# tobwei/APTAI

Measured on AMD Instinct MI355X. Metric: utterances/sec (10 s @ 16 kHz) train-step, higher is better.
Workload: dtype bf16

## Files before the change

### aptai_amd/csrc/attention.hip

```cpp
#include "common.h"

namespace {

#ifdef APTAI_STAMPS
__device__ unsigned long long g_attn_stamps[3 * 1024 * 8];
#define ATTN_STAMP(k, slot)                                                                                       \
    do {                                                                                                          \
        if (threadIdx.x == 0) {                                                                                   \
            const int bl = blockIdx.x + gridDim.x * (blockIdx.y + gridDim.y * blockIdx.z);                        \
            if (bl < 1024) g_attn_stamps[((k) * 1024 + bl) * 8 + (slot)] = wall_clock64();                         \
        }                                                                                                         \
    } while (0)
#else
#define ATTN_STAMP(k, slot) do {} while (0)
#endif

constexpr int HD = 64;
constexpr float LOG2E = 1.4426950408889634f;

struct AttnArgs {
    const bf16_t* qkv; long ld;
    const int* lens;
    bf16_t* ctx; long ldo;
    float* lse2;
// ... 12 lines not shown
    int q_prescaled;
};

__device__ __forceinline__ int tile_swz(int row) { return ((row >> 2) & 3) | (((row >> 1) & 1) << 2); }
__device__ __forceinline__ int tile_off(int row, int chunk) { return row * 128 + ((chunk ^ tile_swz(row)) << 4); }

struct LaneOffs {
    int rowk[4];
    int tr[2][2];
};
__device__ __forceinline__ LaneOffs lane_offs(int lane) {
    LaneOffs o;
    const int r31 = lane & 31, h = lane >> 5;
#pragma unroll
    for (int ds = 0; ds < 4; ++ds) o.rowk[ds] = tile_off(r31, 2 * ds + h);
    const int dgrp = (lane >> 4) & 1, i = lane & 15, qq = i >> 2, p = i & 3;
    const int trow = 4 * h + qq;
#pragma unroll
    for (int dt = 0; dt < 2; ++dt)
#pragma unroll
        for (int hi = 0; hi < 2; ++hi) o.tr[dt][hi] = tile_off(trow + 8 * hi, dt * 4 + 2 * dgrp + (p >> 1)) + ((p & 1) << 3);
    return o;
}
__device__ __forceinline__ bf16x8 rd_row(const char* tile, const LaneOffs& o, int row_block, int ds) {
    return *(const bf16x8*)(tile + o.rowk[ds] + row_block * 4096);
}
__device__ __forceinline__ bf16x8 rd_tr(const char* tile, const LaneOffs& o, int s, int dt) {
    short4v lo = __builtin_amdgcn_ds_read_tr16_b64_v4i16((__attribute__((address_space(3))) short4v*)(tile + o.tr[dt][0] + s * 2048));
    short4v hi = __builtin_amdgcn_ds_read_tr16_b64_v4i16((__attribute__((address_space(3))) short4v*)(tile + o.tr[dt][1] + s * 2048));
    short8v r = {lo[0], lo[1], lo[2], lo[3], hi[0], hi[1], hi[2], hi[3]};
    return __builtin_bit_cast(bf16x8, r);
}

__device__ __forceinline__ bf16x8 pack8(const float* v) {
    u32x4 u = {pack2bf(v[0], v[1]), pack2bf(v[2], v[3]), pack2bf(v[4], v[5]), pack2bf(v[6], v[7])};
    return __builtin_bit_cast(bf16x8, u);
}

__device__ __forceinline__ int acc_row(int r, int h) { return (r & 3) + 8 * (r >> 2) + 4 * h; }

constexpr int OUT_PITCH = 144;
constexpr int STAGE_BYTES = 4 * 32 * OUT_PITCH;
constexpr int DQ_STAGE = 2 * 128 * 128;
constexpr int DKDV_BLOCKS = 3;
constexpr int DKDV_KV_BYTES = 2 * 128 * 128;

__device__ __forceinline__ void stage_rows128(char* dst, const bf16_t* src, long ld, int tid) {
#pragma unroll
    for (int it = 0; it < 4; ++it) {
        const int cid = it * 256 + tid, row = cid >> 3, ch = cid & 7;
        *(u32x4*)(dst + tile_off(row, ch)) = *(const u32x4*)(src + (long)row * ld + ch * 8);
    }
}
__device__ __forceinline__ void store_rows_bf16(char* sw, const f32x16 (&acc)[2], float scale, bf16_t* g_row0, long ld, int lane) {
    const int r31 = lane & 31, h = lane >> 5;
#pragma unroll
    for (int dt = 0; dt < 2; ++dt)
#pragma unroll
        for (int g4 = 0; g4 < 4; ++g4) {
            const int d = dt * 32 + 8 * g4 + 4 * h;
            *(u32x2*)(sw + r31 * OUT_PITCH + d * 2) = (u32x2){pack2bf(acc[dt][4 * g4] * scale, acc[dt][4 * g4 + 1] * scale),
                                                              pack2bf(acc[dt][4 * g4 + 2] * scale, acc[dt][4 * g4 + 3] * scale)};
        }
    __builtin_amdgcn_fence(__ATOMIC_RELEASE, "wavefront");
#pragma unroll
    for (int i = 0; i < 4; ++i) {
        const int idx = i * 64 + lane, r = idx >> 3, ch = idx & 7;
        *(u32x4*)(g_row0 + (long)r * ld + ch * 8) = *(const u32x4*)(sw + r * OUT_PITCH + ch * 16);
    }
    __builtin_amdgcn_fence(__ATOMIC_ACQUIRE, "wavefront");
}

__device__ __forceinline__ bool attn_keep(uint32_t pair, int key, uint32_t s0, uint32_t s1, uint32_t thr16) {
    const uint32_t hsh = rng_hash(pair, s0, s1);
    return ((key & 1) ? (hsh >> 16) : (hsh & 0xffffu)) >= thr16;
}

__device__ __forceinline__ void attn_block(const AttnArgs& a, int& tile, int& hd, int& b) {
    const int nt = gridDim.x, total = nt * gridDim.y * gridDim.z;
    int L = blockIdx.x + nt * (blockIdx.y + gridDim.y * blockIdx.z);
    if (a.xcd_remap && (total & 7) == 0) L = (L & 7) * (total >> 3) + (L >> 3);
    tile = L % nt;
    const int grp = L / nt;
    hd = grp % (int)gridDim.y;
    b = grp / (int)gridDim.y;
}

constexpr int FWD_BUF = 2 * 64 * 128;
constexpr int FWD_SMEM = 2 * FWD_BUF;
constexpr float REF_HEADROOM = 40.0f;
constexpr float REF_SUM_LIMIT = 1.4901161193847656e-08f;

template <bool V> struct Flag { static constexpr bool value = V; };

template <bool DROP>
__global__ __launch_bounds__(256, 3) void attn_fwd_kernel(AttnArgs a) {
    __shared__ __attribute__((aligned(16))) char smem[FWD_SMEM];
    ATTN_STAMP(0, 0);
    if (DROP) apply_salt(a.salt, a.seed0, a.seed1);
    const int tid = threadIdx.x, lane = tid & 63, wave = tid >> 6, h = lane >> 5;
    int tile_x, hd, b;
    attn_block(a, tile_x, hd, b);
    const int q0 = tile_x * 128 + wave * 32;
    int len = a.lens[b];
    len = len < 1 ? 1 : (len > a.Tp ? a.Tp : len);
    const int ntiles = (len + 63) >> 6;
    const long rowbase = (long)b * a.Tp;
    const int q = q0 + (lane & 31);
    const bf16_t* Qg = a.qkv + (rowbase + q) * a.ld + hd * HD;
    const bf16_t* Kg = a.qkv + rowbase * a.ld + a.H + hd * HD;
    const bf16_t* Vg = Kg + a.H;
    const LaneOffs lo = lane_offs(lane);

    bf16x8 qf[4];
#pragma unroll
    for (int ds = 0; ds < 4; ++ds) qf[ds] = *(const bf16x8*)(Qg + ds * 16 + h * 8);
    __builtin_amdgcn_sched_barrier(0);

    f32x16 oT[2];
    oT[0] = (f32x16)(0.f);
    oT[1] = (f32x16)(0.f);
    float ref = 0.f, l_run = 0.f;

    int soff[2];
    long goff[2];
#pragma unroll
    for (int it = 0; it < 2; ++it) {
        const int cid = it * 256 + tid, row = cid >> 3, ch = cid & 7;
        soff[it] = tile_off(row, ch);
        goff[it] = (long)row * a.ld + ch * 8;
    }
    u32x4 kreg[2], vreg[2];
    const long tile_stride = 64 * a.ld;
#pragma unroll
    for (int it = 0; it < 2; ++it) { kreg[it] = *(const u32x4*)(Kg + goff[it]); vreg[it] = *(const u32x4*)(Vg + goff[it]); }
    uint32_t hbase = 0;
    if (DROP) hbase = rng_hash((uint32_t)((b * a.heads + hd) * a.Tp + q), a.seed0, a.seed1) + (uint32_t)(2 * h) * ATTN_K1;
    const float c = a.c;
#pragma unroll
    for (int it = 0; it < 2; ++it) { *(u32x4*)(smem + soff[it]) = kreg[it]; *(u32x4*)(smem + 64 * 128 + soff[it]) = vreg[it]; }
    if (ntiles > 1) {
#pragma unroll
        for (int it = 0; it < 2; ++it) {
            kreg[it] = *(const u32x4*)(Kg + tile_stride + goff[it]);
            vreg[it] = *(const u32x4*)(Vg + tile_stride + goff[it]);
        }
    }
    __syncthreads();
    ATTN_STAMP(0, 1);

    auto tile = [&](auto first_flag, auto mask_flag, const int t) {
        constexpr bool FIRST = decltype(first_flag)::value, MASK = decltype(mask_flag)::value;
        const char* sK = smem + (t & 1) * FWD_BUF;
        const char* sV = sK + 64 * 128;
        const int kbase = t * 64;
        bf16x8 kfr[2][4];
#pragma unroll
        for (int ds = 0; ds < 4; ++ds) kfr[0][ds] = rd_row(sK, lo, 0, ds);
        if (t + 1 < ntiles) {
            char* nb = smem + ((t + 1) & 1) * FWD_BUF;
#pragma unroll
            for (int it = 0; it < 2; ++it) { *(u32x4*)(nb + soff[it]) = kreg[it]; *(u32x4*)(nb + 64 * 128 + soff[it]) = vreg[it]; }
            if (t + 2 < ntiles) {
                const bf16_t* kn = Kg + (long)(t + 2) * tile_stride;
                const bf16_t* vn = Vg + (long)(t + 2) * tile_stride;
#pragma unroll
                for (int it = 0; it < 2; ++it) { kreg[it] = *(const u32x4*)(kn + goff[it]); vreg[it] = *(const u32x4*)(vn + goff[it]); }
            }
        }
        f32x16 sT[2];
        sT[0] = __builtin_amdgcn_mfma_f32_32x32x16_bf16(kfr[0][0], qf[0], (f32x16)(0.f), 0, 0, 0);
#pragma unroll
        for (int ds = 1; ds < 4; ++ds) sT[0] = __builtin_amdgcn_mfma_f32_32x32x16_bf16(kfr[0][ds], qf[ds], sT[0], 0, 0, 0);
#pragma unroll
        for (int ds = 0; ds < 4; ++ds) kfr[1][ds] = rd_row(sK, lo, 1, ds);
        sT[1] = __builtin_amdgcn_mfma_f32_32x32x16_bf16(kfr[1][0], qf[0], (f32x16)(0.f), 0, 0, 0);
#pragma unroll
        for (int ds = 1; ds < 4; ++ds) sT[1] = __builtin_amdgcn_mfma_f32_32x32x16_bf16(kfr[1][ds], qf[ds], sT[1], 0, 0, 0);
        if (MASK) {
#pragma unroll
            for (int kt2 = 0; kt2 < 2; ++kt2)
#pragma unroll
                for (int r = 0; r < 16; ++r)
                    if (kbase + kt2 * 32 + acc_row(r, h) >= len) sT[kt2][r] = -INFINITY;
        }
        if (FIRST) {
            float mt = sT[0][0];
#pragma unroll
            for (int r = 1; r < 16; ++r) mt = fmaxf(mt, sT[0][r]);
#pragma unroll
            for (int r = 0; r < 16; ++r) mt = fmaxf(mt, sT[1][r]);
            mt = fmaxf(mt, __shfl_xor(mt, 32, 64));
            ref = fmaf(mt, c, REF_HEADROOM);
        }
        float psum = 0.f;
#pragma unroll
        for (int kt2 = 0; kt2 < 2; ++kt2) {
            bf16x8 vfr[2][2];
#pragma unroll
            for (int s = 0; s < 2; ++s)
#pragma unroll
                for (int dt = 0; dt < 2; ++dt) vfr[s][dt] = rd_tr(sV, lo, 2 * kt2 + s, dt);
            float x[16];
#pragma unroll
            for (int r = 0; r < 16; ++r) { x[r] = fast_exp2(fmaf(sT[kt2][r], c, -ref)); psum += x[r]; }
            if (DROP) {
#pragma unroll
                for (int r = 0; r < 16; r += 2) {
                    const uint32_t hsh = attn_mix(hbase + (uint32_t)(kbase / 2 + 16 * kt2 + acc_row(r, 0) / 2) * ATTN_K1);
                    x[r] = (hsh & 0xffffu) >= a.thr16 ? x[r] : 0.f;
                    x[r + 1] = (hsh >> 16) >= a.thr16 ? x[r + 1] : 0.f;
                }
            }
            const bf16x8 pf0 = pack8(&x[0]), pf1 = pack8(&x[8]);
#pragma unroll
            for (int dt = 0; dt < 2; ++dt) oT[dt] = __builtin_amdgcn_mfma_f32_32x32x16_bf16(vfr[0][dt], pf0, oT[dt], 0, 0, 0);
#pragma unroll
            for (int dt = 0; dt < 2; ++dt) oT[dt] = __builtin_amdgcn_mfma_f32_32x32x16_bf16(vfr[1][dt], pf1, oT[dt], 0, 0, 0);
        }
        psum += __shfl_xor(psum, 32, 64);
        l_run += psum;
        if (!FIRST && __builtin_amdgcn_ballot_w64(!(psum <= REF_SUM_LIMIT))) {
            if (!(psum <= REF_SUM_LIMIT)) {
                const float e = floorf(fast_log2(psum)) + REF_HEADROOM;
                const float sc = fast_exp2(-e);
                ref += e;
                l_run *= sc;
#pragma unroll
                for (int r = 0; r < 16; ++r) { oT[0][r] *= sc; oT[1][r] *= sc; }
            }
        }
        __syncthreads();
    };
    if (ntiles == 1) {
        tile(Flag<true>{}, Flag<true>{}, 0);
    } else {
        tile(Flag<true>{}, Flag<false>{}, 0);
        for (int t = 1; t + 1 < ntiles; ++t) tile(Flag<false>{}, Flag<false>{}, t);
        tile(Flag<false>{}, Flag<true>{}, ntiles - 1);
    }
    ATTN_STAMP(0, 2);
    const float l_tot = l_run;
    const float inv = __frcp_rn(l_tot) * a.dscale;
    if (a.lse2 && h == 0) a.lse2[((long)b * a.heads + hd) * a.Tp + q] = ref + fast_log2(l_tot);
    char* sw = smem + wave * (32 * OUT_PITCH);
    const int r31 = lane & 31;
#pragma unroll
    for (int dt = 0; dt < 2; ++dt)
#pragma unroll
        for (int g4 = 0; g4 < 4; ++g4) {
            oT[dt][4 * g4 + 0] *= inv; oT[dt][4 * g4 + 1] *= inv; oT[dt][4 * g4 + 2] *= inv; oT[dt][4 * g4 + 3] *= inv;
            const int d = dt * 32 + 8 * g4 + 4 * h;
            *(u32x2*)(sw + r31 * OUT_PITCH + d * 2) = (u32x2){pack2bf(oT[dt][4 * g4], oT[dt][4 * g4 + 1]),
                                                              pack2bf(oT[dt][4 * g4 + 2], oT[dt][4 * g4 + 3])};
        }
    __syncthreads();
    const long orow = (rowbase + q0) * a.ldo + hd * HD;
#pragma unroll
    for (int i = 0; i < 4; ++i) {
        const int idx = i * 64 + lane, r = idx >> 3, ch = idx & 7;
        *(u32x4*)(a.ctx + orow + (long)r * a.ldo + ch * 8) = *(const u32x4*)(sw + r * OUT_PITCH + ch * 16);
    }
    if (a.o32) {
#pragma unroll
        for (int dt = 0; dt < 2; ++dt) {
            __syncthreads();
#pragma unroll
            for (int g4 = 0; g4 < 4; ++g4)
                *(f32x4*)(sw + r31 * OUT_PITCH + (8 * g4 + 4 * h) * 4) =
                    (f32x4){oT[dt][4 * g4], oT[dt][4 * g4 + 1], oT[dt][4 * g4 + 2], oT[dt][4 * g4 + 3]};
            __syncthreads();
#pragma unroll
            for (int i = 0; i < 4; ++i) {
                const int idx = i * 64 + lane, r = idx >> 3, ch = idx & 7;
                *(f32x4*)(a.o32 + orow + (long)r * a.ldo + dt * 32 + ch * 4) = *(const f32x4*)(sw + r * OUT_PITCH + ch * 16);
            }
        }
    }
    ATTN_STAMP(0, 3);
#ifdef APTAI_STAMPS
    asm volatile("s_waitcnt vmcnt(0)" ::: "memory");
    ATTN_STAMP(0, 4);
#endif
}

template <bool PRE>
__global__ __launch_bounds__(256, PRE ? DKDV_BLOCKS : 2) void attn_bwd_dkdv_kernel(AttnArgs a) {
    __shared__ __attribute__((aligned(16))) char smem[STAGE_BYTES + 384 + DKDV_KV_BYTES];
    char* sQ = smem;
    char* sD = smem + 32 * 128;
    float* sL = (float*)(smem + STAGE_BYTES);
    char* sKall = smem + STAGE_BYTES + 384;
    char* sVall = sKall + 128 * 128;
    ATTN_STAMP(1, 0);
    if (a.thr16) apply_salt(a.salt, a.seed0, a.seed1);
    const int tid = threadIdx.x, lane = tid & 63, wave = tid >> 6, h = lane >> 5;
    int tile_x, hd, b;
    attn_block(a, tile_x, hd, b);
    const int kb0 = tile_x * 128;
    const int key0 = kb0 + wave * 32;
    int len = a.lens[b];
    len = len < 1 ? 1 : (len > a.Tp ? a.Tp : len);
    const long rowbase = (long)b * a.Tp;
    const int key = key0 + (lane & 31);
    bf16_t* dK0 = a.dqkv + (rowbase + kb0) * a.ld + a.H + hd * HD;
    bf16_t* dV0 = dK0 + a.H;
    if (kb0 >= len) {
        const u32x4 z = {0u, 0u, 0u, 0u};
#pragma unroll
        for (int it = 0; it < 4; ++it) {
            const int cid = it * 256 + tid, row = cid >> 3, ch = cid & 7;
            *(u32x4*)(dK0 + (long)row * a.ld + ch * 8) = z;
            *(u32x4*)(dV0 + (long)row * a.ld + ch * 8) = z;
        }
        return;
    }
    const LaneOffs lo = lane_offs(lane);
    const bf16_t* K0 = a.qkv + (rowbase + kb0) * a.ld + a.H + hd * HD;
    stage_rows128(sKall, K0, a.ld, tid);
    stage_rows128(sVall, K0 + a.H, a.ld, tid);
    f32x16 dKT[2], dVT[2];
    dKT[0] = dKT[1] = dVT[0] = dVT[1] = (f32x16)(0.f);

    const int nq = a.skip_pad_q ? ((len + 31) >> 5) : (a.Tp >> 5);
    const bf16_t* Qb = a.qkv + rowbase * a.ld + hd * HD;
    const bf16_t* Db = a.dctx + rowbase * a.ldo + hd * HD;
    const float* lse = a.lse2 + ((long)b * a.heads + hd) * a.Tp;
    const float* del = a.delta + ((long)b * a.heads + hd) * a.Tp;
    const int srow = tid >> 3, sch = tid & 7;
    const int soff = tile_off(srow, sch);
    const long gq = (long)srow * a.ld + sch * 8, gd = (long)srow * a.ldo + sch * 8;
    u32x4 qreg = *(const u32x4*)(Qb + gq), dreg = *(const u32x4*)(Db + gd);
    const float* stat = (tid < 8 ? lse : del) + (tid & 7) * 4;
    f32x4 sreg = (f32x4)(0.f);
    if (tid < 16) sreg = *(const f32x4*)stat;
    const bool key_ok = key < len;
    const bool wave_boundary = key0 + 32 > len;
    const uint32_t hshift = (key & 1) ? 16u : 0u;
    const float c = a.c;
    const uint32_t pairk = (uint32_t)(key >> 1) * ATTN_K1;
    const uint32_t rowid0 = (uint32_t)((b * a.heads + hd) * a.Tp) + (uint32_t)(tid & 31);
    uint32_t hreg = 0;
    if (a.thr16 && tid >= 32 && tid < 64) hreg = rng_hash(rowid0, a.seed0, a.seed1);
    ATTN_STAMP(1, 1);
    for (int t = 0; t < nq; ++t) {
        __syncthreads();
        *(u32x4*)(sQ + soff) = qreg;
        *(u32x4*)(sD + soff) = dreg;
        if (tid < 16) *(f32x4*)(sL + tid * 4) = PRE ? -sreg : sreg;
        if (a.thr16 && tid >= 32 && tid < 64) ((uint32_t*)sL)[64 + (tid & 31)] = hreg;
        __syncthreads();
        if (t + 1 < nq) {
            qreg = *(const u32x4*)(Qb + (long)(t + 1) * 32 * a.ld + gq);
            dreg = *(const u32x4*)(Db + (long)(t + 1) * 32 * a.ldo + gd);
            if (tid < 16) sreg = *(const f32x4*)(stat + (t + 1) * 32);
            if (a.thr16 && tid >= 32 && tid < 64) hreg = rng_hash(rowid0 + (uint32_t)((t + 1) * 32), a.seed0, a.seed1);
        }
        f32x16 cs = (f32x16)(0.f), cd = (f32x16)(0.f);
        if (PRE) {
#pragma unroll
            for (int g4 = 0; g4 < 4; ++g4) {
                const f32x4 l4 = *(const f32x4*)(sL + 8 * g4 + 4 * h);
                const f32x4 d4 = *(const f32x4*)(sL + 32 + 8 * g4 + 4 * h);
#pragma unroll
                for (int rr = 0; rr < 4; ++rr) { cs[4 * g4 + rr] = l4[rr]; cd[4 * g4 + rr] = d4[rr]; }
            }
        }
        f32x16 s = __builtin_amdgcn_mfma_f32_32x32x16_bf16(rd_row(sQ, lo, 0, 0), rd_row(sKall, lo, wave, 0), cs, 0, 0, 0);
        f32x16 dp = __builtin_amdgcn_mfma_f32_32x32x16_bf16(rd_row(sD, lo, 0, 0), rd_row(sVall, lo, wave, 0), cd, 0, 0, 0);
#pragma unroll
        for (int ds = 1; ds < 4; ++ds) {
            s = __builtin_amdgcn_mfma_f32_32x32x16_bf16(rd_row(sQ, lo, 0, ds), rd_row(sKall, lo, wave, ds), s, 0, 0, 0);
            dp = __builtin_amdgcn_mfma_f32_32x32x16_bf16(rd_row(sD, lo, 0, ds), rd_row(sVall, lo, wave, ds), dp, 0, 0, 0);
        }
        float pd[16], dsv[16];
        if (PRE) {
#pragma unroll
            for (int r = 0; r < 16; ++r) pd[r] = fast_exp2(s[r]);
        } else {
#pragma unroll
            for (int g4 = 0; g4 < 4; ++g4) {
                const f32x4 l4 = *(const f32x4*)(sL + 8 * g4 + 4 * h);
                const f32x4 d4 = *(const f32x4*)(sL + 32 + 8 * g4 + 4 * h);
#pragma unroll
                for (int rr = 0; rr < 4; ++rr) {
                    pd[4 * g4 + rr] = fast_exp2(fmaf(s[4 * g4 + rr], c, -l4[rr]));
                    dsv[4 * g4 + rr] = d4[rr];
                }
            }
        }
        if (wave_boundary) {
#pragma unroll
            for (int r = 0; r < 16; ++r) pd[r] = key_ok ? pd[r] : 0.f;
        }
        if (a.thr16) {
#pragma unroll
            for (int g4 = 0; g4 < 4; ++g4) {
                const u32x4 rh = *(const u32x4*)((const uint32_t*)sL + 64 + 8 * g4 + 4 * h);
                f32x4 nd4 = (f32x4)(0.f);
                if (PRE) nd4 = *(const f32x4*)(sL + 32 + 8 * g4 + 4 * h);
#pragma unroll
                for (int rr = 0; rr < 4; ++rr) {
                    const int r = 4 * g4 + rr;
                    const uint32_t y = attn_mix(rh[rr] + pairk);
                    const bool k = ((y >> hshift) & 0xffffu) >= a.thr16;
                    const float p0 = pd[r];
                    if (PRE) dsv[r] = p0 * (k ? dp[r] : nd4[rr]);
                    else dsv[r] = p0 * ((k ? dp[r] : 0.f) - dsv[r]);
                    pd[r] = k ? p0 : 0.f;
                }
            }
        } else {
#pragma unroll
            for (int r = 0; r < 16; ++r) dsv[r] = PRE ? pd[r] * dp[r] : pd[r] * (dp[r] - dsv[r]);
        }
#pragma unroll
        for (int sstep = 0; sstep < 2; ++sstep) {
            const bf16x8 pf = pack8(&pd[8 * sstep]);
            const bf16x8 df = pack8(&dsv[8 * sstep]);
#pragma unroll
            for (int dt = 0; dt < 2; ++dt) {
                dVT[dt] = __builtin_amdgcn_mfma_f32_32x32x16_bf16(rd_tr(sD, lo, sstep, dt), pf, dVT[dt], 0, 0, 0);
                dKT[dt] = __builtin_amdgcn_mfma_f32_32x32x16_bf16(rd_tr(sQ, lo, sstep, dt), df, dKT[dt], 0, 0, 0);
            }
        }
    }
    __syncthreads();
    ATTN_STAMP(1, 2);
    char* sw = smem + wave * (32 * OUT_PITCH);
    store_rows_bf16(sw, dKT, (PRE ? 0.6931471805599453f : a.scale) * a.dscale, dK0 + (long)(wave * 32) * a.ld, a.ld, lane);
    store_rows_bf16(sw, dVT, a.dscale, dV0 + (long)(wave * 32) * a.ld, a.ld, lane);
    ATTN_STAMP(1, 3);
#ifdef APTAI_STAMPS
    asm volatile("s_waitcnt vmcnt(0)" ::: "memory");
    ATTN_STAMP(1, 4);
#endif
}

template <bool PRE>
__global__ __launch_bounds__(256, 3) void attn_bwd_dq_kernel(AttnArgs a) {
    __shared__ __attribute__((aligned(16))) char smem[DQ_STAGE + 512];
    char* sK = smem;
    char* sV = smem + 32 * 128;
    float* sDel = (float*)(smem + DQ_STAGE);
    ATTN_STAMP(2, 0);
    if (a.thr16) apply_salt(a.salt, a.seed0, a.seed1);
    const int tid = threadIdx.x, lane = tid & 63, wave = tid >> 6, h = lane >> 5;
    int tile_x, hd, b;
    attn_block(a, tile_x, hd, b);
    const int qb0 = tile_x * 128;
    const int q = qb0 + wave * 32 + (lane & 31);
    int len = a.lens[b];
    len = len < 1 ? 1 : (len > a.Tp ? a.Tp : len);
    const long rowbase = (long)b * a.Tp;
    const LaneOffs lo = lane_offs(lane);
    bf16x8 qf[4], df[4];
    const bf16_t* Kb = a.qkv + rowbase * a.ld + a.H + hd * HD;
    const bf16_t* Vb = Kb + a.H;
    const int srow = tid >> 3, sch = tid & 7;
    const int soff = tile_off(srow, sch);
    const long gk = (long)srow * a.ld + sch * 8;
    u32x4 kreg = *(const u32x4*)(Kb + gk), vreg = *(const u32x4*)(Vb + gk);
    const bf16_t* Qrows = a.qkv + (rowbase + qb0) * a.ld + hd * HD;
    const bf16_t* Drows = a.dctx + (rowbase + qb0) * a.ldo + hd * HD;
    u32x4 qst[4], dst[4];
#pragma unroll
    for (int it = 0; it < 4; ++it) {
        const int cid = it * 256 + tid, row = cid >> 3, ch = cid & 7;
        qst[it] = *(const u32x4*)(Qrows + (long)row * a.ld + ch * 8);
        dst[it] = *(const u32x4*)(Drows + (long)row * a.ldo + ch * 8);
    }
    const int part = lane & 15, rsub = lane >> 4;
    f32x4 ovv[8];
#pragma unroll
    for (int it = 0; it < 8; ++it) {
        const int row = wave * 32 + it * 4 + rsub;
        const long g = (rowbase + qb0 + row) * a.ldo + hd * HD + part * 4;
        if (a.o32) {
            ovv[it] = *(const f32x4*)(a.o32 + g);
        } else {
            const u32x2 ov = *(const u32x2*)(a.ctx + g);
            ovv[it] = (f32x4){lo_bf(ov[0]), hi_bf(ov[0]), lo_bf(ov[1]), hi_bf(ov[1])};
        }
    }
    const float lse_q = a.lse2[((long)b * a.heads + hd) * a.Tp + q];
    char* sQt = smem;
    char* sDt = smem + 128 * 128;
#pragma unroll
    for (int it = 0; it < 4; ++it) {
        const int cid = it * 256 + tid, row = cid >> 3, ch = cid & 7;
        *(u32x4*)(sQt + tile_off(row, ch)) = qst[it];
        *(u32x4*)(sDt + tile_off(row, ch)) = dst[it];
    }
    ATTN_STAMP(2, 5);
    __syncthreads();
    ATTN_STAMP(2, 6);
#pragma unroll
    for (int ds = 0; ds < 4; ++ds) { qf[ds] = rd_row(sQt, lo, wave, ds); df[ds] = rd_row(sDt, lo, wave, ds); }
#pragma unroll
    for (int it = 0; it < 8; ++it) {
        const int row = wave * 32 + it * 4 + rsub;
        const u32x2 dv = *(const u32x2*)(sDt + tile_off(row, part >> 1) + ((part & 1) << 3));
        float acc = lo_bf(dv[0]) * ovv[it][0];
        acc = fmaf(hi_bf(dv[0]), ovv[it][1], acc);
        acc = fmaf(lo_bf(dv[1]), ovv[it][2], acc);
        acc = fmaf(hi_bf(dv[1]), ovv[it][3], acc);
        acc += __shfl_xor(acc, 8, 64);
        acc += __shfl_xor(acc, 4, 64);
        acc += __shfl_xor(acc, 2, 64);
        acc += __shfl_xor(acc, 1, 64);
        if (part == 0) sDel[row] = acc;
    }
    ATTN_STAMP(2, 7);
    __syncthreads();
    float del_q = sDel[wave * 32 + (lane & 31)];
    __syncthreads();
    del_q *= __frcp_rn(a.dscale);
    if (h == 0) a.delta[((long)b * a.heads + hd) * a.Tp + q] = del_q;
    f32x16 dQT[2];
    dQT[0] = dQT[1] = (f32x16)(0.f);
    const int nk = (len + 31) >> 5;
    uint32_t hbase = 0;
    if (a.thr16) hbase = rng_hash((uint32_t)((b * a.heads + hd) * a.Tp + q), a.seed0, a.seed1) + (uint32_t)(2 * h) * ATTN_K1;
    const float c = a.c;
    const f32x16 cs = (f32x16)(PRE ? -lse_q : 0.f), cd = (f32x16)(PRE ? -del_q : 0.f);
    ATTN_STAMP(2, 1);
    for (int t = 0; t < nk; ++t) {
        __syncthreads();
        *(u32x4*)(sK + soff) = kreg;
        *(u32x4*)(sV + soff) = vreg;
        __syncthreads();
        if (t + 1 < nk) {
            kreg = *(const u32x4*)(Kb + (long)(t + 1) * 32 * a.ld + gk);
            vreg = *(const u32x4*)(Vb + (long)(t + 1) * 32 * a.ld + gk);
        }
        f32x16 sT = __builtin_amdgcn_mfma_f32_32x32x16_bf16(rd_row(sK, lo, 0, 0), qf[0], cs, 0, 0, 0);
        f32x16 dpT = __builtin_amdgcn_mfma_f32_32x32x16_bf16(rd_row(sV, lo, 0, 0), df[0], cd, 0, 0, 0);
#pragma unroll
        for (int ds = 1; ds < 4; ++ds) {
            sT = __builtin_amdgcn_mfma_f32_32x32x16_bf16(rd_row(sK, lo, 0, ds), qf[ds], sT, 0, 0, 0);
            dpT = __builtin_amdgcn_mfma_f32_32x32x16_bf16(rd_row(sV, lo, 0, ds), df[ds], dpT, 0, 0, 0);
        }
        float dsv[16];
        const bool boundary = t * 32 + 32 > len;
#pragma unroll
        for (int r = 0; r < 16; ++r) {
            float p = PRE ? fast_exp2(sT[r]) : fast_exp2(fmaf(sT[r], c, -lse_q));
            if (boundary && (t * 32 + acc_row(r, h) >= len)) p = 0.f;
            dsv[r] = p;
        }
        if (a.thr16) {
            const float dropped = PRE ? -del_q : 0.f;
#pragma unroll
            for (int r = 0; r < 16; r += 2) {
                const uint32_t hsh = attn_mix(hbase + (uint32_t)(t * 16 + acc_row(r, 0) / 2) * ATTN_K1);
                dpT[r] = (hsh & 0xffffu) >= a.thr16 ? dpT[r] : dropped;
                dpT[r + 1] = (hsh >> 16) >= a.thr16 ? dpT[r + 1] : dropped;
            }
        }
#pragma unroll
        for (int r = 0; r < 16; ++r) dsv[r] *= PRE ? dpT[r] : (dpT[r] - del_q);
#pragma unroll
        for (int sstep = 0; sstep < 2; ++sstep) {
            const bf16x8 dsf = pack8(&dsv[8 * sstep]);
#pragma unroll
            for (int dt = 0; dt < 2; ++dt)
                dQT[dt] = __builtin_amdgcn_mfma_f32_32x32x16_bf16(rd_tr(sK, lo, sstep, dt), dsf, dQT[dt], 0, 0, 0);
        }
    }
    __syncthreads();
    ATTN_STAMP(2, 2);
    store_rows_bf16(smem + wave * (32 * OUT_PITCH), dQT, a.scale * a.dscale,
                    a.dqkv + (rowbase + qb0 + wave * 32) * a.ld + hd * HD, a.ld, lane);
    ATTN_STAMP(2, 3);
#ifdef APTAI_STAMPS
    asm volatile("s_waitcnt vmcnt(0)" ::: "memory");
    ATTN_STAMP(2, 4);
#endif
}

__device__ __forceinline__ uint32_t lds_u32x(const char* p) {
    return (uint32_t)(uintptr_t)(__attribute__((address_space(3))) const char*)p;
}

struct AttnXArgs {
    const bf16_t* qkv; long ld;
    const int* lens;
    bf16_t* ctx; long ldo;
    int B, Tp, H, heads, slots;
    float c;
    int xcd_remap;
};

__device__ __forceinline__ void tr_pair_asm(uint32_t a_lo, uint32_t a_hi, short4v& lo, short4v& hi) {
    asm volatile("ds_read_b64_tr_b16 %0, %1" : "=v"(lo) : "v"(a_lo));
    asm volatile("ds_read_b64_tr_b16 %0, %1" : "=v"(hi) : "v"(a_hi));
}
__device__ __forceinline__ bf16x8 tr_join(const short4v lo, const short4v hi) {
    return __builtin_bit_cast(bf16x8, (short8v){lo[0], lo[1], lo[2], lo[3], hi[0], hi[1], hi[2], hi[3]});
}
template <int NPQ>
__device__ __forceinline__ void split8(const float* x, bf16x8 (&out)[NPQ]) {
    u32x4 hq, mq, lq;
    float r1[8];
#pragma unroll
    for (int i = 0; i < 4; ++i) {
        hq[i] = pack2bf(x[2 * i], x[2 * i + 1]);
        r1[2 * i] = x[2 * i] - lo_bf(hq[i]);
        r1[2 * i + 1] = x[2 * i + 1] - hi_bf(hq[i]);
        mq[i] = pack2bf(r1[2 * i], r1[2 * i + 1]);
        if (NPQ == 3) lq[i] = pack2bf(r1[2 * i] - lo_bf(mq[i]), r1[2 * i + 1] - hi_bf(mq[i]));
    }
    out[0] = __builtin_bit_cast(bf16x8, hq);
    out[1] = __builtin_bit_cast(bf16x8, mq);
    if constexpr (NPQ == 3) out[2] = __builtin_bit_cast(bf16x8, lq);
}

template <int NPQ>
__global__ __launch_bounds__(256, NPQ == 2 ? 2 : 1) void attn_exact_fwd_kernel(AttnXArgs a) {
    extern __shared__ __attribute__((aligned(16))) char xsmem[];
    constexpr int TILE = 64 * 128;
    constexpr int STAGE = 2 * NPQ * TILE;
    constexpr int NPROD = NPQ == 2 ? 3 : 6;
    constexpr int PA[6] = {0, 0, 1, 1, 0, 2}, PB[6] = {0, 1, 0, 1, 2, 0};
    constexpr int ASLOT[3] = {0, 2, 5}, BSLOT[3] = {0, 1, 4};
    const int tid = threadIdx.x, lane = tid & 63, wave = tid >> 6, h = lane >> 5;
    const int nt = gridDim.x, total = nt * gridDim.y * gridDim.z;
    int L = blockIdx.x + nt * (blockIdx.y + gridDim.y * blockIdx.z);
    if (a.xcd_remap && (total & 7) == 0) L = (L & 7) * (total >> 3) + (L >> 3);
    const int tile_x = L % nt, grp = L / nt, hd = grp % (int)gridDim.y, b = grp / (int)gridDim.y;
    const int q0 = tile_x * 128 + wave * 32;
    int len = a.lens[b];
    len = len < 1 ? 1 : (len > a.Tp ? a.Tp : len);
// ... 54 lines not shown
                for (int s = 0; s < 2; ++s)
#pragma unroll
                    for (int dt = 0; dt < 2; ++dt)
                        tr_pair_asm(vbase + (uint32_t)(j * TILE + (2 * kt2 + s) * 2048 + lo.tr[dt][0]),
                                    vbase + (uint32_t)(j * TILE + (2 * kt2 + s) * 2048 + lo.tr[dt][1]), vl[j][s][dt], vh[j][s][dt]);
            f32x16 sT = (f32x16)(0.f);
#pragma unroll
            for (int ds = 0; ds < 4; ++ds) {
                bf16x8 kfr[NPQ];
#pragma unroll
                for (int j = 0; j < NPQ; ++j) kfr[j] = rd_row(sK + j * TILE, lo, kt2, ds);
#pragma unroll
                for (int pr = NPROD - 1; pr >= 0; --pr)
                    sT = __builtin_amdgcn_mfma_f32_32x32x16_bf16(kfr[PB[pr]], qf[PA[pr]][ds], sT, 0, 0, 0);
            }
            if (MASK) {
#pragma unroll
                for (int r = 0; r < 16; ++r)
                    if (kbase + kt2 * 32 + acc_row(r, h) >= len) sT[r] = -INFINITY;
            }
            if (FIRST && kt2 == 0) {
                float mt = sT[0];
#pragma unroll
                for (int r = 1; r < 16; ++r) mt = fmaxf(mt, sT[r]);
                mt = fmaxf(mt, __shfl_xor(mt, 32, 64));
                ref = fmaf(mt, c, REF_HEADROOM);
            }
            float x[16];
#pragma unroll
            for (int r = 0; r < 16; ++r) { x[r] = fast_exp2(fmaf(sT[r], c, -ref)); psum += x[r]; }
            bf16x8 pf[2][NPQ];
            split8<NPQ>(&x[0], pf[0]);
            split8<NPQ>(&x[8], pf[1]);
            asm volatile("s_waitcnt lgkmcnt(0)" ::: "memory");
#pragma unroll
            for (int j = 0; j < NPQ; ++j)
#pragma unroll
                for (int s = 0; s < 2; ++s)
                    asm volatile("" : "+v"(vl[j][s][0]), "+v"(vh[j][s][0]), "+v"(vl[j][s][1]), "+v"(vh[j][s][1]));
#pragma unroll
            for (int s = 0; s < 2; ++s)
#pragma unroll
                for (int pr = NPROD - 1; pr >= 0; --pr)
#pragma unroll
                    for (int dt = 0; dt < 2; ++dt)
                        oT[dt] = __builtin_amdgcn_mfma_f32_32x32x16_bf16(tr_join(vl[PB[pr]][s][dt], vh[PB[pr]][s][dt]), pf[s][PA[pr]],
                                                                         oT[dt], 0, 0, 0);
        }
        psum += __shfl_xor(psum, 32, 64);
        l_run += psum;
        if (!FIRST && __builtin_amdgcn_ballot_w64(!(psum <= REF_SUM_LIMIT))) {
            if (!(psum <= REF_SUM_LIMIT)) {
                const float e = floorf(fast_log2(psum)) + REF_HEADROOM;
                const float sc = fast_exp2(-e);
                ref += e;
                l_run *= sc;
#pragma unroll
                for (int r = 0; r < 16; ++r) { oT[0][r] *= sc; oT[1][r] *= sc; }
            }
        }
    };
    for (int t = 0; t < ntiles; ++t) {
        asm volatile("s_waitcnt vmcnt(0)" ::: "memory");
        __syncthreads();
        if (t + 1 < ntiles) issue(t + 1);
        const bool last = t + 1 == ntiles;
        if (t == 0) { if (last) tile(Flag<true>{}, Flag<true>{}, 0); else tile(Flag<true>{}, Flag<false>{}, 0); }
        else if (last) tile(Flag<false>{}, Flag<true>{}, t);
        else tile(Flag<false>{}, Flag<false>{}, t);
// ... 538 lines not shown
```

Measured before the change: 1724.

## Stream attention K/V/Q/dO tiles via direct global-to-LDS DMA with async transposed reads

The forward, dK/dV and dQ attention kernels stop staging tiles through registers and instead use global_load_lds DMA, with the swizzle applied to the global address, into double-buffered LDS slots. The trailing per-tile barrier is replaced by a vmcnt wait plus one barrier before issuing the next tile. Transposed V/K/Q/dO reads become inline-asm ds_read_b64_tr_b16 with immediate offsets and explicit lgkmcnt waits, so they overlap the softmax and pack math. The dK/dV kernel also DMAs the lse/delta statistics, and the dQ kernel unrolls by slot and applies the boundary mask only on the last tile. This aims to cut VGPR pressure and register-to-LDS store traffic, at the cost of fragile hand-placed wait counts and an extra vmcnt stall on every tile.

```diff
diff --git a/aptai_amd/csrc/attention.hip b/aptai_amd/csrc/attention.hip
--- a/aptai_amd/csrc/attention.hip
+++ b/aptai_amd/csrc/attention.hip
@@ -68,6 +68,37 @@
     return __builtin_bit_cast(bf16x8, r);
 }
 
+__device__ __forceinline__ uint32_t lds_u32x(const char* p) {
+    return (uint32_t)(uintptr_t)(__attribute__((address_space(3))) const char*)p;
+}
+__device__ __forceinline__ void tr_pair_asm(uint32_t a_lo, uint32_t a_hi, short4v& lo, short4v& hi) {
+    asm volatile("ds_read_b64_tr_b16 %0, %1" : "=&v"(lo) : "v"(a_lo));
+    asm volatile("ds_read_b64_tr_b16 %0, %1" : "=&v"(hi) : "v"(a_hi));
+}
+template <int OFF>
+__device__ __forceinline__ void tr_pair_asm_at(uint32_t a_lo, uint32_t a_hi, short4v& lo, short4v& hi) {
+    static_assert(OFF >= 0 && OFF < 65536, "ds offset field");
+    asm volatile("ds_read_b64_tr_b16 %0, %1 offset:%2" : "=&v"(lo) : "v"(a_lo), "n"(OFF));
+    asm volatile("ds_read_b64_tr_b16 %0, %1 offset:%2" : "=&v"(hi) : "v"(a_hi), "n"(OFF));
+}
+__device__ __forceinline__ bf16x8 tr_join(const short4v lo, const short4v hi) {
+    return __builtin_bit_cast(bf16x8, (short8v){lo[0], lo[1], lo[2], lo[3], hi[0], hi[1], hi[2], hi[3]});
+}
+#define ATTN_TR_WAIT(N, L0, H0, L1, H1) asm volatile("s_waitcnt lgkmcnt(" #N ")" : "+v"(L0), "+v"(H0), "+v"(L1), "+v"(H1)::"memory")
+__device__ __forceinline__ const char* uniform_ptr(const void* p) {
+    const uint64_t u = (uint64_t)p;
+    uint32_t lo = (uint32_t)__builtin_amdgcn_readfirstlane((int)(uint32_t)u), hi = (uint32_t)__builtin_amdgcn_readfirstlane((int)(u >> 32));
+    asm("" : "+s"(lo), "+s"(hi));
+    return (const char*)(((uint64_t)hi << 32) | lo);
+}
+__device__ __forceinline__ void dma16(const bf16_t* base, uint32_t lane_bytes, char* lds) {
+    asm("" : "+v"(lane_bytes));
+    __builtin_amdgcn_global_load_lds(GLB_PTR(uniform_ptr(base) + lane_bytes), LDS_PTR(lds), 16, 0, 0);
+}
+
+template <bool V> struct Flag { static constexpr bool value = V; };
+template <int V> struct Int { static constexpr int value = V; };
+
 __device__ __forceinline__ bf16x8 pack8(const float* v) {
     u32x4 u = {pack2bf(v[0], v[1]), pack2bf(v[2], v[3]), pack2bf(v[4], v[5]), pack2bf(v[6], v[7])};
     return __builtin_bit_cast(bf16x8, u);
@@ -78,6 +109,9 @@
 constexpr int OUT_PITCH = 144;
 constexpr int STAGE_BYTES = 4 * 32 * OUT_PITCH;
 constexpr int DQ_STAGE = 2 * 128 * 128;
+constexpr int DQ_SLOT = 2 * 32 * 128;
+constexpr int DKDV_SLOT = 2 * 32 * 128;
+constexpr int DKDV_STAT = 384;
 constexpr int DKDV_BLOCKS = 3;
 constexpr int DKDV_KV_BYTES = 2 * 128 * 128;
 
@@ -126,8 +160,6 @@
 constexpr int FWD_SMEM = 2 * FWD_BUF;
 constexpr float REF_HEADROOM = 40.0f;
 constexpr float REF_SUM_LIMIT = 1.4901161193847656e-08f;
-
-template <bool V> struct Flag { static constexpr bool value = V; };
 
 template <bool DROP>
 __global__ __launch_bounds__(256, 3) void attn_fwd_kernel(AttnArgs a) {
@@ -158,52 +190,44 @@
     oT[1] = (f32x16)(0.f);
     float ref = 0.f, l_run = 0.f;
 
-    int soff[2];
-    long goff[2];
+    uint32_t goff[2];
 #pragma unroll
     for (int it = 0; it < 2; ++it) {
-        const int cid = it * 256 + tid, row = cid >> 3, ch = cid & 7;
-        soff[it] = tile_off(row, ch);
-        goff[it] = (long)row * a.ld + ch * 8;
-    }
-    u32x4 kreg[2], vreg[2];
+        const int cid = it * 256 + tid, row = cid >> 3, cp = cid & 7;
+        goff[it] = 2u * ((uint32_t)row * (uint32_t)a.ld + (uint32_t)((cp ^ tile_swz(row)) << 3));
+    }
     const long tile_stride = 64 * a.ld;
-#pragma unroll
-    for (int it = 0; it < 2; ++it) { kreg[it] = *(const u32x4*)(Kg + goff[it]); vreg[it] = *(const u32x4*)(Vg + goff[it]); }
+    auto issue = [&](int t) {
+        char* dst = smem + (t & 1) * FWD_BUF + __builtin_amdgcn_readfirstlane(wave) * 1024;
+#pragma unroll
+        for (int it = 0; it < 2; ++it) {
+            dma16(Kg + (long)t * tile_stride, goff[it], dst + it * 4096);
+            dma16(Vg + (long)t * tile_stride, goff[it], dst + 64 * 128 + it * 4096);
+        }
+    };
+    issue(0);
     uint32_t hbase = 0;
     if (DROP) hbase = rng_hash((uint32_t)((b * a.heads + hd) * a.Tp + q), a.seed0, a.seed1) + (uint32_t)(2 * h) * ATTN_K1;
     const float c = a.c;
-#pragma unroll
-    for (int it = 0; it < 2; ++it) { *(u32x4*)(smem + soff[it]) = kreg[it]; *(u32x4*)(smem + 64 * 128 + soff[it]) = vreg[it]; }
-    if (ntiles > 1) {
-#pragma unroll
-        for (int it = 0; it < 2; ++it) {
-            kreg[it] = *(const u32x4*)(Kg + tile_stride + goff[it]);
-            vreg[it] = *(const u32x4*)(Vg + tile_stride + goff[it]);
-        }
-    }
-    __syncthreads();
+    uint32_t tra[2][2];
+#pragma unroll
+    for (int dt = 0; dt < 2; ++dt)
+#pragma unroll
+        for (int hi = 0; hi < 2; ++hi) tra[dt][hi] = lds_u32x(smem) + (uint32_t)(64 * 128 + lo.tr[dt][hi]);
     ATTN_STAMP(0, 1);
 
     auto tile = [&](auto first_flag, auto mask_flag, const int t) {
         constexpr bool FIRST = decltype(first_flag)::value, MASK = decltype(mask_flag)::value;
-        const char* sK = smem + (t & 1) * FWD_BUF;
-        const char* sV = sK + 64 * 128;
+        const int so = (t & 1) * FWD_BUF;
+        const char* sK = smem + so;
         const int kbase = t * 64;
+        asm volatile("s_waitcnt vmcnt(0)" ::: "memory");
+        __syncthreads();
+        if (t + 1 < ntiles) issue(t + 1);
+        const uint32_t ta[2][2] = {{tra[0][0] + so, tra[0][1] + so}, {tra[1][0] + so, tra[1][1] + so}};
         bf16x8 kfr[2][4];
 #pragma unroll
         for (int ds = 0; ds < 4; ++ds) kfr[0][ds] = rd_row(sK, lo, 0, ds);
-        if (t + 1 < ntiles) {
-            char* nb = smem + ((t + 1) & 1) * FWD_BUF;
-#pragma unroll
-            for (int it = 0; it < 2; ++it) { *(u32x4*)(nb + soff[it]) = kreg[it]; *(u32x4*)(nb + 64 * 128 + soff[it]) = vreg[it]; }
-            if (t + 2 < ntiles) {
-                const bf16_t* kn = Kg + (long)(t + 2) * tile_stride;
-                const bf16_t* vn = Vg + (long)(t + 2) * tile_stride;
-#pragma unroll
-                for (int it = 0; it < 2; ++it) { kreg[it] = *(const u32x4*)(kn + goff[it]); vreg[it] = *(const u32x4*)(vn + goff[it]); }
-            }
-        }
         f32x16 sT[2];
         sT[0] = __builtin_amdgcn_mfma_f32_32x32x16_bf16(kfr[0][0], qf[0], (f32x16)(0.f), 0, 0, 0);
 #pragma unroll
@@ -232,11 +256,18 @@
         float psum = 0.f;
 #pragma unroll
         for (int kt2 = 0; kt2 < 2; ++kt2) {
-            bf16x8 vfr[2][2];
-#pragma unroll
-            for (int s = 0; s < 2; ++s)
-#pragma unroll
-                for (int dt = 0; dt < 2; ++dt) vfr[s][dt] = rd_tr(sV, lo, 2 * kt2 + s, dt);
+            short4v vl[4], vh[4];
+            if (kt2 == 0) {
+                tr_pair_asm_at<0>(ta[0][0], ta[0][1], vl[0], vh[0]);
+                tr_pair_asm_at<0>(ta[1][0], ta[1][1], vl[1], vh[1]);
+                tr_pair_asm_at<2048>(ta[0][0], ta[0][1], vl[2], vh[2]);
+                tr_pair_asm_at<2048>(ta[1][0], ta[1][1], vl[3], vh[3]);
+            } else {
+                tr_pair_asm_at<4096>(ta[0][0], ta[0][1], vl[0], vh[0]);
+                tr_pair_asm_at<4096>(ta[1][0], ta[1][1], vl[1], vh[1]);
+                tr_pair_asm_at<6144>(ta[0][0], ta[0][1], vl[2], vh[2]);
+                tr_pair_asm_at<6144>(ta[1][0], ta[1][1], vl[3], vh[3]);
+            }
             float x[16];
 #pragma unroll
             for (int r = 0; r < 16; ++r) { x[r] = fast_exp2(fmaf(sT[kt2][r], c, -ref)); psum += x[r]; }
@@ -249,10 +280,12 @@
                 }
             }
             const bf16x8 pf0 = pack8(&x[0]), pf1 = pack8(&x[8]);
-#pragma unroll
-            for (int dt = 0; dt < 2; ++dt) oT[dt] = __builtin_amdgcn_mfma_f32_32x32x16_bf16(vfr[0][dt], pf0, oT[dt], 0, 0, 0);
-#pragma unroll
-            for (int dt = 0; dt < 2; ++dt) oT[dt] = __builtin_amdgcn_mfma_f32_32x32x16_bf16(vfr[1][dt], pf1, oT[dt], 0, 0, 0);
+            ATTN_TR_WAIT(0, vl[0], vh[0], vl[1], vh[1]);
+            ATTN_TR_WAIT(0, vl[2], vh[2], vl[3], vh[3]);
+#pragma unroll
+            for (int dt = 0; dt < 2; ++dt) oT[dt] = __builtin_amdgcn_mfma_f32_32x32x16_bf16(tr_join(vl[dt], vh[dt]), pf0, oT[dt], 0, 0, 0);
+#pragma unroll
+            for (int dt = 0; dt < 2; ++dt) oT[dt] = __builtin_amdgcn_mfma_f32_32x32x16_bf16(tr_join(vl[2 + dt], vh[2 + dt]), pf1, oT[dt], 0, 0, 0);
         }
         psum += __shfl_xor(psum, 32, 64);
         l_run += psum;
@@ -266,7 +299,6 @@
                 for (int r = 0; r < 16; ++r) { oT[0][r] *= sc; oT[1][r] *= sc; }
             }
         }
-        __syncthreads();
     };
     if (ntiles == 1) {
         tile(Flag<true>{}, Flag<true>{}, 0);
@@ -275,6 +307,7 @@
         for (int t = 1; t + 1 < ntiles; ++t) tile(Flag<false>{}, Flag<false>{}, t);
         tile(Flag<false>{}, Flag<true>{}, ntiles - 1);
     }
+    __syncthreads();
     ATTN_STAMP(0, 2);
     const float l_tot = l_run;
     const float inv = __frcp_rn(l_tot) * a.dscale;
@@ -322,11 +355,9 @@
 
 template <bool PRE>
 __global__ __launch_bounds__(256, PRE ? DKDV_BLOCKS : 2) void attn_bwd_dkdv_kernel(AttnArgs a) {
-    __shared__ __attribute__((aligned(16))) char smem[STAGE_BYTES + 384 + DKDV_KV_BYTES];
-    char* sQ = smem;
-    char* sD = smem + 32 * 128;
-    float* sL = (float*)(smem + STAGE_BYTES);
-    char* sKall = smem + STAGE_BYTES + 384;
+    __shared__ __attribute__((aligned(16))) char smem[STAGE_BYTES + 2 * DKDV_STAT + DKDV_KV_BYTES];
+    static_assert(2 * DKDV_SLOT <= STAGE_BYTES, "the ring lives in the staging area");
+    char* sKall = smem + STAGE_BYTES + 2 * DKDV_STAT;
     char* sVall = sKall + 128 * 128;
     ATTN_STAMP(1, 0);
     if (a.thr16) apply_salt(a.salt, a.seed0, a.seed1);
@@ -352,45 +383,67 @@
         return;
     }
     const LaneOffs lo = lane_offs(lane);
+    const int nq = a.skip_pad_q ? ((len + 31) >> 5) : (a.Tp >> 5);
+    const bf16_t* Qb = a.qkv + rowbase * a.ld + hd * HD;
+    const bf16_t* Db = a.dctx + rowbase * a.ldo + hd * HD;
+    const float* lse = a.lse2 + ((long)b * a.heads + hd) * a.Tp;
+    const float* del = a.delta + ((long)b * a.heads + hd) * a.Tp;
+    const int srow = tid >> 3, sch = (tid & 7) ^ tile_swz(srow);
+    const uint32_t gq = 2u * ((uint32_t)srow * (uint32_t)a.ld + sch * 8), gd = 2u * ((uint32_t)srow * (uint32_t)a.ldo + sch * 8);
+    auto issue = [&](int t, int slot) {
+        char* dst = smem + slot * DKDV_SLOT + __builtin_amdgcn_readfirstlane(wave) * 1024;
+        dma16(Qb + (long)t * 32 * a.ld, gq, dst);
+        dma16(Db + (long)t * 32 * a.ldo, gd, dst + 32 * 128);
+    };
+    issue(0, 0);
     const bf16_t* K0 = a.qkv + (rowbase + kb0) * a.ld + a.H + hd * HD;
     stage_rows128(sKall, K0, a.ld, tid);
     stage_rows128(sVall, K0 + a.H, a.ld, tid);
     f32x16 dKT[2], dVT[2];
     dKT[0] = dKT[1] = dVT[0] = dVT[1] = (f32x16)(0.f);
 
-    const int nq = a.skip_pad_q ? ((len + 31) >> 5) : (a.Tp >> 5);
-    const bf16_t* Qb = a.qkv + rowbase * a.ld + hd * HD;
-    const bf16_t* Db = a.dctx + rowbase * a.ldo + hd * HD;
-    const float* lse = a.lse2 + ((long)b * a.heads + hd) * a.Tp;
-    const float* del = a.delta + ((long)b * a.heads + hd) * a.Tp;
-    const int srow = tid >> 3, sch = tid & 7;
-    const int soff = tile_off(srow, sch);
-    const long gq = (long)srow * a.ld + sch * 8, gd = (long)srow * a.ldo + sch * 8;
-    u32x4 qreg = *(const u32x4*)(Qb + gq), dreg = *(const u32x4*)(Db + gd);
-    const float* stat = (tid < 8 ? lse : del) + (tid & 7) * 4;
-    f32x4 sreg = (f32x4)(0.f);
-    if (tid < 16) sreg = *(const f32x4*)stat;
     const bool key_ok = key < len;
     const bool wave_boundary = key0 + 32 > len;
     const uint32_t hshift = (key & 1) ? 16u : 0u;
     const float c = a.c;
     const uint32_t pairk = (uint32_t)(key >> 1) * ATTN_K1;
     const uint32_t rowid0 = (uint32_t)((b * a.heads + hd) * a.Tp) + (uint32_t)(tid & 31);
-    uint32_t hreg = 0;
-    if (a.thr16 && tid >= 32 && tid < 64) hreg = rng_hash(rowid0, a.seed0, a.seed1);
+    static_assert(2 * DKDV_SLOT + 2 * 256 <= STAGE_BYTES, "raw statistics slots");
+    auto raw_issue = [&](int t) {
+        char* dst = smem + 2 * DKDV_SLOT + (t & 1) * 256;
+        uint32_t lb = (uint32_t)(tid & 31) * 4u;
+        asm("" : "+v"(lb));
+        if (tid < 32) __builtin_amdgcn_global_load_lds(GLB_PTR(uniform_ptr(lse + t * 32) + lb), LDS_PTR(dst), 4, 0, 0);
+        else __builtin_amdgcn_global_load_lds(GLB_PTR(uniform_ptr(del + t * 32) + lb), LDS_PTR(dst), 4, 0, 0);
+    };
+    auto put_stats = [&](int t, float v) {
+        float* sl = (float*)(smem + STAGE_BYTES + (t & 1) * DKDV_STAT);
+        sl[tid] = PRE ? -v : v;
+        if (a.thr16 && tid >= 32) ((uint32_t*)sl)[64 + (tid & 31)] = rng_hash(rowid0 + (uint32_t)(t * 32), a.seed0, a.seed1);
+    };
+    if (tid < 64) {
+        if (nq > 1) raw_issue(1);
+        put_stats(0, tid < 32 ? lse[tid] : del[tid & 31]);
+    }
+    uint32_t tra[2][2];
+#pragma unroll
+    for (int dt = 0; dt < 2; ++dt)
+#pragma unroll
+        for (int hi = 0; hi < 2; ++hi) tra[dt][hi] = lds_u32x(smem) + (uint32_t)lo.tr[dt][hi];
     ATTN_STAMP(1, 1);
-    for (int t = 0; t < nq; ++t) {
-        __syncthreads();
-        *(u32x4*)(sQ + soff) = qreg;
-        *(u32x4*)(sD + soff) = dreg;
-        if (tid < 16) *(f32x4*)(sL + tid * 4) = PRE ? -sreg : sreg;
-        if (a.thr16 && tid >= 32 && tid < 64) ((uint32_t*)sL)[64 + (tid & 31)] = hreg;
+    auto tile = [&](const int t) {
+        const int slot = t & 1, so = slot * DKDV_SLOT;
+        const char* sQ = smem + so;
+        const char* sD = sQ + 32 * 128;
+        const float* sL = (const float*)(smem + STAGE_BYTES + slot * DKDV_STAT);
+        const uint32_t ta[2][2] = {{tra[0][0] + so, tra[0][1] + so}, {tra[1][0] + so, tra[1][1] + so}};
+        asm volatile("s_waitcnt vmcnt(0)" ::: "memory");
         __syncthreads();
         if (t + 1 < nq) {
-            qreg = *(const u32x4*)(Qb + (long)(t + 1) * 32 * a.ld + gq);
-            dreg = *(const u32x4*)(Db + (long)(t + 1) * 32 * a.ldo + gd);
-            if (tid < 16) sreg = *(const f32x4*)(stat + (t + 1) * 32);
-            if (a.thr16 && tid >= 32 && tid < 64) hreg = rng_hash(rowid0 + (uint32_t)((t + 1) * 32), a.seed0, a.seed1);
+            if (tid < 64) put_stats(t + 1, *(const float*)(smem + 2 * DKDV_SLOT + (slot ^ 1) * 256 + tid * 4));
+            __builtin_amdgcn_sched_barrier(0);
+            issue(t + 1, slot ^ 1);
+            if (t + 2 < nq && tid < 64) raw_issue(t + 2);
         }
         f32x16 cs = (f32x16)(0.f), cd = (f32x16)(0.f);
         if (PRE) {
@@ -450,17 +503,33 @@
 #pragma unroll
             for (int r = 0; r < 16; ++r) dsv[r] = PRE ? pd[r] * dp[r] : pd[r] * (dp[r] - dsv[r]);
         }
-#pragma unroll
-        for (int sstep = 0; sstep < 2; ++sstep) {
-            const bf16x8 pf = pack8(&pd[8 * sstep]);
-            const bf16x8 df = pack8(&dsv[8 * sstep]);
-#pragma unroll
-            for (int dt = 0; dt < 2; ++dt) {
-                dVT[dt] = __builtin_amdgcn_mfma_f32_32x32x16_bf16(rd_tr(sD, lo, sstep, dt), pf, dVT[dt], 0, 0, 0);
-                dKT[dt] = __builtin_amdgcn_mfma_f32_32x32x16_bf16(rd_tr(sQ, lo, sstep, dt), df, dKT[dt], 0, 0, 0);
-            }
-        }
-    }
+        short4v fl[2][4], fh[2][4];
+        const bf16x8 pf0 = pack8(&pd[0]), df0 = pack8(&dsv[0]);
+        tr_pair_asm_at<4096>(ta[0][0], ta[0][1], fl[0][0], fh[0][0]);
+        tr_pair_asm_at<0>(ta[0][0], ta[0][1], fl[0][2], fh[0][2]);
+        tr_pair_asm_at<4096>(ta[1][0], ta[1][1], fl[0][1], fh[0][1]);
+        tr_pair_asm_at<0>(ta[1][0], ta[1][1], fl[0][3], fh[0][3]);
+        const bf16x8 pf1 = pack8(&pd[8]), df1 = pack8(&dsv[8]);
+        tr_pair_asm_at<6144>(ta[0][0], ta[0][1], fl[1][0], fh[1][0]);
+        tr_pair_asm_at<2048>(ta[0][0], ta[0][1], fl[1][2], fh[1][2]);
+        tr_pair_asm_at<6144>(ta[1][0], ta[1][1], fl[1][1], fh[1][1]);
+        tr_pair_asm_at<2048>(ta[1][0], ta[1][1], fl[1][3], fh[1][3]);
+        ATTN_TR_WAIT(8, fl[0][0], fh[0][0], fl[0][1], fh[0][1]);
+        ATTN_TR_WAIT(8, fl[0][2], fh[0][2], fl[0][3], fh[0][3]);
+#pragma unroll
+        for (int dt = 0; dt < 2; ++dt) {
+            dVT[dt] = __builtin_amdgcn_mfma_f32_32x32x16_bf16(tr_join(fl[0][dt], fh[0][dt]), pf0, dVT[dt], 0, 0, 0);
+            dKT[dt] = __builtin_amdgcn_mfma_f32_32x32x16_bf16(tr_join(fl[0][2 + dt], fh[0][2 + dt]), df0, dKT[dt], 0, 0, 0);
+        }
+        ATTN_TR_WAIT(0, fl[1][0], fh[1][0], fl[1][1], fh[1][1]);
+        ATTN_TR_WAIT(0, fl[1][2], fh[1][2], fl[1][3], fh[1][3]);
+#pragma unroll
+        for (int dt = 0; dt < 2; ++dt) {
+            dVT[dt] = __builtin_amdgcn_mfma_f32_32x32x16_bf16(tr_join(fl[1][dt], fh[1][dt]), pf1, dVT[dt], 0, 0, 0);
+            dKT[dt] = __builtin_amdgcn_mfma_f32_32x32x16_bf16(tr_join(fl[1][2 + dt], fh[1][2 + dt]), df1, dKT[dt], 0, 0, 0);
+        }
+    };
+    for (int t = 0; t < nq; ++t) tile(t);
     __syncthreads();
     ATTN_STAMP(1, 2);
     char* sw = smem + wave * (32 * OUT_PITCH);
@@ -476,8 +545,6 @@
 template <bool PRE>
 __global__ __launch_bounds__(256, 3) void attn_bwd_dq_kernel(AttnArgs a) {
     __shared__ __attribute__((aligned(16))) char smem[DQ_STAGE + 512];
-    char* sK = smem;
-    char* sV = smem + 32 * 128;
     float* sDel = (float*)(smem + DQ_STAGE);
     ATTN_STAMP(2, 0);
     if (a.thr16) apply_salt(a.salt, a.seed0, a.seed1);
@@ -493,10 +560,13 @@
     bf16x8 qf[4], df[4];
     const bf16_t* Kb = a.qkv + rowbase * a.ld + a.H + hd * HD;
     const bf16_t* Vb = Kb + a.H;
-    const int srow = tid >> 3, sch = tid & 7;
-    const int soff = tile_off(srow, sch);
-    const long gk = (long)srow * a.ld + sch * 8;
-    u32x4 kreg = *(const u32x4*)(Kb + gk), vreg = *(const u32x4*)(Vb + gk);
+    const int srow = tid >> 3;
+    const uint32_t gk = 2u * ((uint32_t)srow * (uint32_t)a.ld + (uint32_t)(((tid & 7) ^ tile_swz(srow)) << 3));
+    auto issue = [&](int t, int slot) {
+        char* dst = smem + slot * DQ_SLOT + __builtin_amdgcn_readfirstlane(wave) * 1024;
+        dma16(Kb + (long)t * 32 * a.ld, gk, dst);
+        dma16(Vb + (long)t * 32 * a.ld, gk, dst + 32 * 128);
+    };
     const bf16_t* Qrows = a.qkv + (rowbase + qb0) * a.ld + hd * HD;
     const bf16_t* Drows = a.dctx + (rowbase + qb0) * a.ldo + hd * HD;
     u32x4 qst[4], dst[4];
@@ -550,7 +620,7 @@
     ATTN_STAMP(2, 7);
     __syncthreads();
     float del_q = sDel[wave * 32 + (lane & 31)];
-    __syncthreads();
+    issue(0, 0);
     del_q *= __frcp_rn(a.dscale);
     if (h == 0) a.delta[((long)b * a.heads + hd) * a.Tp + q] = del_q;
     f32x16 dQT[2];
@@ -561,15 +631,20 @@
     const float c = a.c;
     const f32x16 cs = (f32x16)(PRE ? -lse_q : 0.f), cd = (f32x16)(PRE ? -del_q : 0.f);
     ATTN_STAMP(2, 1);
-    for (int t = 0; t < nk; ++t) {
+    uint32_t tra[2][2];
+#pragma unroll
+    for (int dt = 0; dt < 2; ++dt)
+#pragma unroll
+        for (int hi = 0; hi < 2; ++hi) tra[dt][hi] = lds_u32x(smem) + (uint32_t)lo.tr[dt][hi];
+    auto tile = [&](auto slot_c, auto last_c, const int t) {
+        constexpr int SLOT = decltype(slot_c)::value;
+        constexpr bool LAST = decltype(last_c)::value;
+        constexpr int SBASE = SLOT * DQ_SLOT;
+        const char* sK = smem + SBASE;
+        const char* sV = sK + 32 * 128;
+        asm volatile("s_waitcnt vmcnt(0)" ::: "memory");
         __syncthreads();
-        *(u32x4*)(sK + soff) = kreg;
-        *(u32x4*)(sV + soff) = vreg;
-        __syncthreads();
-        if (t + 1 < nk) {
-            kreg = *(const u32x4*)(Kb + (long)(t + 1) * 32 * a.ld + gk);
-            vreg = *(const u32x4*)(Vb + (long)(t + 1) * 32 * a.ld + gk);
-        }
+        if (t + 1 < nk) issue(t + 1, SLOT ^ 1);
         f32x16 sT = __builtin_amdgcn_mfma_f32_32x32x16_bf16(rd_row(sK, lo, 0, 0), qf[0], cs, 0, 0, 0);
         f32x16 dpT = __builtin_amdgcn_mfma_f32_32x32x16_bf16(rd_row(sV, lo, 0, 0), df[0], cd, 0, 0, 0);
 #pragma unroll
@@ -578,11 +653,10 @@
             dpT = __builtin_amdgcn_mfma_f32_32x32x16_bf16(rd_row(sV, lo, 0, ds), df[ds], dpT, 0, 0, 0);
         }
         float dsv[16];
-        const bool boundary = t * 32 + 32 > len;
 #pragma unroll
         for (int r = 0; r < 16; ++r) {
             float p = PRE ? fast_exp2(sT[r]) : fast_exp2(fmaf(sT[r], c, -lse_q));
-            if (boundary && (t * 32 + acc_row(r, h) >= len)) p = 0.f;
+            if (LAST && (t * 32 + acc_row(r, h) >= len)) p = 0.f;
             dsv[r] = p;
         }
         if (a.thr16) {
@@ -594,14 +668,35 @@
                 dpT[r + 1] = (hsh >> 16) >= a.thr16 ? dpT[r + 1] : dropped;
             }
         }
-#pragma unroll
-        for (int r = 0; r < 16; ++r) dsv[r] *= PRE ? dpT[r] : (dpT[r] - del_q);
-#pragma unroll
-        for (int sstep = 0; sstep < 2; ++sstep) {
-            const bf16x8 dsf = pack8(&dsv[8 * sstep]);
-#pragma unroll
-            for (int dt = 0; dt < 2; ++dt)
-                dQT[dt] = __builtin_amdgcn_mfma_f32_32x32x16_bf16(rd_tr(sK, lo, sstep, dt), dsf, dQT[dt], 0, 0, 0);
+        short4v kl[4], kh[4];
+#pragma unroll
+        for (int r = 0; r < 8; ++r) dsv[r] *= PRE ? dpT[r] : (dpT[r] - del_q);
+        const bf16x8 dsf0 = pack8(&dsv[0]);
+        tr_pair_asm_at<SBASE>(tra[0][0], tra[0][1], kl[0], kh[0]);
+        tr_pair_asm_at<SBASE>(tra[1][0], tra[1][1], kl[1], kh[1]);
+#pragma unroll
+        for (int r = 8; r < 16; ++r) dsv[r] *= PRE ? dpT[r] : (dpT[r] - del_q);
+        const bf16x8 dsf1 = pack8(&dsv[8]);
+        tr_pair_asm_at<SBASE + 2048>(tra[0][0], tra[0][1], kl[2], kh[2]);
+        tr_pair_asm_at<SBASE + 2048>(tra[1][0], tra[1][1], kl[3], kh[3]);
+        ATTN_TR_WAIT(4, kl[0], kh[0], kl[1], kh[1]);
+        dQT[0] = __builtin_amdgcn_mfma_f32_32x32x16_bf16(tr_join(kl[0], kh[0]), dsf0, dQT[0], 0, 0, 0);
+        dQT[1] = __builtin_amdgcn_mfma_f32_32x32x16_bf16(tr_join(kl[1], kh[1]), dsf0, dQT[1], 0, 0, 0);
+        ATTN_TR_WAIT(0, kl[2], kh[2], kl[3], kh[3]);
+        dQT[0] = __builtin_amdgcn_mfma_f32_32x32x16_bf16(tr_join(kl[2], kh[2]), dsf1, dQT[0], 0, 0, 0);
+        dQT[1] = __builtin_amdgcn_mfma_f32_32x32x16_bf16(tr_join(kl[3], kh[3]), dsf1, dQT[1], 0, 0, 0);
+    };
+    {
+        int t = 0;
+        for (; t + 2 < nk; t += 2) {
+            tile(Int<0>{}, Flag<false>{}, t);
+            tile(Int<1>{}, Flag<false>{}, t + 1);
+        }
+        if (t + 2 == nk) {
+            tile(Int<0>{}, Flag<false>{}, t);
+            tile(Int<1>{}, Flag<true>{}, t + 1);
+        } else {
+            tile(Int<0>{}, Flag<true>{}, t);
         }
     }
     __syncthreads();
@@ -615,10 +710,6 @@
 #endif
 }
 
-__device__ __forceinline__ uint32_t lds_u32x(const char* p) {
-    return (uint32_t)(uintptr_t)(__attribute__((address_space(3))) const char*)p;
-}
-
 struct AttnXArgs {
     const bf16_t* qkv; long ld;
     const int* lens;
@@ -628,13 +719,6 @@
     int xcd_remap;
 };
 
-__device__ __forceinline__ void tr_pair_asm(uint32_t a_lo, uint32_t a_hi, short4v& lo, short4v& hi) {
-    asm volatile("ds_read_b64_tr_b16 %0, %1" : "=v"(lo) : "v"(a_lo));
-    asm volatile("ds_read_b64_tr_b16 %0, %1" : "=v"(hi) : "v"(a_hi));
-}
-__device__ __forceinline__ bf16x8 tr_join(const short4v lo, const short4v hi) {
-    return __builtin_bit_cast(bf16x8, (short8v){lo[0], lo[1], lo[2], lo[3], hi[0], hi[1], hi[2], hi[3]});
-}
 template <int NPQ>
 __device__ __forceinline__ void split8(const float* x, bf16x8 (&out)[NPQ]) {
     u32x4 hq, mq, lq;
@@ -755,9 +839,11 @@
             bf16x8 pf[2][NPQ];
             split8<NPQ>(&x[0], pf[0]);
             split8<NPQ>(&x[8], pf[1]);
-            asm volatile("s_waitcnt lgkmcnt(0)" ::: "memory");
-#pragma unroll
-            for (int j = 0; j < NPQ; ++j)
+            asm volatile("s_waitcnt lgkmcnt(0)"
+                         : "+v"(vl[0][0][0]), "+v"(vh[0][0][0]), "+v"(vl[0][0][1]), "+v"(vh[0][0][1]), "+v"(vl[0][1][0]), "+v"(vh[0][1][0]),
+                           "+v"(vl[0][1][1]), "+v"(vh[0][1][1])::"memory");
+#pragma unroll
+            for (int j = 1; j < NPQ; ++j)
 #pragma unroll
                 for (int s = 0; s < 2; ++s)
                     asm volatile("" : "+v"(vl[j][s][0]), "+v"(vh[j][s][0]), "+v"(vl[j][s][1]), "+v"(vh[j][s][1]));
```

After: 1716. Within noise of the previous version (-0.5%).
